# frederik-kofoed-marqversen/quantum_computations

Measured on AMD Instinct MI355X. Metric: gate_apps_per_sec, higher is better.
Workload: dtype f64; 1 GPU; 28-qubit complex128 state vector (28 qubits = 4 GiB per GPU), depth-100 random 1+2-qubit gates (BASELINE.json configs[1], seed 100); n_qubits=28

## Files before the change

quantum_computations_amd/csrc/qsv_api.hip:

```cpp

#include "qsv_internal.h"
#include "qsv_plan.h"

#include <sys/mman.h>

#include <thread>

#include <cmath>
#include <cstring>
#include <vector>

namespace {

thread_local std::string g_last_error;

bool valid(const qsv_state *st) { return st != nullptr; }

inline int bit_of(const qsv_state *st, int q) { return st->n - 1 - q; }

int check_qubits(const qsv_state *st, int k, const int *qs) {
    if (st->kind != 0) return qsv_fail(QSV_ESTATE, "this call needs a qubit register");
    for (int i = 0; i < k; ++i) {
        if (qs[i] < 0) return qsv_fail(QSV_EINVAL, "Non-negative index");
        if (qs[i] >= st->n)
            return qsv_fail(QSV_EINVAL, "qubit index " + std::to_string(qs[i]) + " out of range for a " +
                                            std::to_string(st->n) + "-qubit register");
        for (int j = 0; j < i; ++j)
            if (qs[i] == qs[j]) return qsv_fail(QSV_EINVAL, "Indices must be distinct.");
    }
    return QSV_OK;
}

int alloc_workspace(qsv_state *st) {
    QSV_HIP(hipMalloc(reinterpret_cast<void **>(&st->partials), sizeof(double) * 2 * QSV_REDUCE_BLOCKS));
    QSV_HIP(hipHostMalloc(reinterpret_cast<void **>(&st->partials_host), sizeof(double) * 2 * QSV_REDUCE_BLOCKS,
                          hipHostMallocDefault));
    QSV_HIP(hipEventCreate(&st->ev_start));
    QSV_HIP(hipEventCreate(&st->ev_stop));
    return QSV_OK;
}

int create_common(int kind, int n, int d, uint64_t amps, int device, void *dev_amps, uint64_t capacity,
                  void *stream, qsv_state **out) {
    if (!out) return qsv_fail(QSV_EINVAL, "null output handle");
    *out = nullptr;
    int count = 0;
    hipError_t e = hipGetDeviceCount(&count);
    if (e != hipSuccess || count <= 0)
        return qsv_fail(QSV_EHIP, std::string("no HIP device available: ") +
                                      (e != hipSuccess ? hipGetErrorString(e) : "device count is 0"));
    if (device < 0 || device >= count) return qsv_fail(QSV_EINVAL, "device ordinal out of range");
    QSV_HIP(hipSetDevice(device));
    qsv_state *st = new qsv_state();
    st->device = device;
    st->kind = kind;
    st->n = n;
    st->d = d;
    st->amps = amps;
    st->stream = static_cast<hipStream_t>(stream);
    if (dev_amps) {
        if (capacity < amps) {
            delete st;
            return qsv_fail(QSV_ENOMEM, "view capacity is smaller than the register");
        }
        st->data = static_cast<amp_t *>(dev_amps);
        st->capacity = capacity;
        st->owns_data = false;
    } else {
        if (hipMalloc(reinterpret_cast<void **>(&st->data), sizeof(amp_t) * amps) != hipSuccess) {
            delete st;
            return qsv_fail(QSV_ENOMEM, "device allocation of " + std::to_string(amps * sizeof(amp_t)) +
                                            " bytes for the register failed");
        }
        st->capacity = amps;
        st->owns_data = true;
    }
    int rc = alloc_workspace(st);
    if (rc) {
        qsv_destroy(st);
        return rc;
    }
    if (st->owns_data) {
        rc = qsvk_set_basis(st, 0);
        if (rc) {
            qsv_destroy(st);
            return rc;
        }
    }
    *out = st;
    return QSV_OK;
}

bool is_one(double re, double im) { return re == 1.0 && im == 0.0; }
bool is_zero(double re, double im) { return re == 0.0 && im == 0.0; }

bool matrix_is_diagonal(int D, const double *m) {
    for (int r = 0; r < D; ++r)
        for (int c = 0; c < D; ++c)
            if (r != c && !is_zero(m[2 * (r * D + c)], m[2 * (r * D + c) + 1])) return false;
    return true;
}

bool matrix_equals(int D, const double *m, const double *ref_real) {
    for (int i = 0; i < D * D; ++i)
        if (m[2 * i] != ref_real[i] || m[2 * i + 1] != 0.0) return false;
    return true;
}

constexpr int QSV_MIN_CTRL_BIT = 3;

constexpr int OP_NONE = -1;

QsvOp dense_op(int k, const int *bits, int nctrl, const int *cbits, const double *m) {
    QsvOp op;
    op.kind = QSV_OP_DENSE;
    op.k = k;
    for (int j = 0; j < k; ++j) op.bits[j] = bits[j];
    op.nctrl = nctrl;
    for (int i = 0; i < nctrl; ++i) op.cbits[i] = cbits[i];
    std::memcpy(op.m, m, sizeof(double) * (2u << (2 * k)));
    return op;
}

QsvOp diag_op(int k, const int *bits, int nctrl, const int *cbits, const double *d) {
    QsvOp op;
    op.kind = QSV_OP_DIAG;
    op.k = k;
    for (int j = 0; j < k; ++j) op.bits[j] = bits[j];
    op.nctrl = nctrl;
    for (int i = 0; i < nctrl; ++i) op.cbits[i] = cbits[i];
    std::memcpy(op.m, d, sizeof(double) * (2u << k));
    return op;
}

QsvOp phase_op(int nctrl, const int *cbits, double re, double im) {
    QsvOp op;
    op.kind = QSV_OP_PHASE;
    op.nctrl = nctrl;
    for (int i = 0; i < nctrl; ++i) op.cbits[i] = cbits[i];
    op.m[0] = re;
    op.m[1] = im;
    return op;
}

QsvOp none_op() {
    QsvOp op;
    op.kind = OP_NONE;
    return op;
}

QsvOp diag_1q_bits(qsv_state *st, int bit, const double d[4]) {
    if (st->specialize && is_one(d[0], d[1])) {
        if (is_one(d[2], d[3])) return none_op();
        if (bit >= QSV_MIN_CTRL_BIT) return phase_op(1, &bit, d[2], d[3]);
    }
    return diag_op(1, &bit, 0, nullptr, d);
}

QsvOp diag_2q_bits(qsv_state *st, int b0, int b1, const double d[8]) {
    if (st->specialize) {
        const bool one0 = is_one(d[0], d[1]), one1 = is_one(d[2], d[3]), one2 = is_one(d[4], d[5]);
        const bool c0 = b0 >= QSV_MIN_CTRL_BIT, c1 = b1 >= QSV_MIN_CTRL_BIT;
        if (one0 && one1 && one2) {
            if (is_one(d[6], d[7])) return none_op();
            const double dd[4] = {1.0, 0.0, d[6], d[7]};
            if (c0 && c1) {
                const int both[2] = {b0, b1};
                return phase_op(2, both, d[6], d[7]);
            }
            if (c0) return diag_op(1, &b1, 1, &b0, dd);
            if (c1) return diag_op(1, &b0, 1, &b1, dd);
        } else if (one0 && one1 && c0) {
            return diag_op(1, &b1, 1, &b0, d + 4);
        } else if (one0 && one2 && d[2] == d[6] && d[3] == d[7]) {
            const double dd[4] = {1.0, 0.0, d[2], d[3]};
            return diag_1q_bits(st, b1, dd);
        }
    }
    const int bits[2] = {b0, b1};
    return diag_op(2, bits, 0, nullptr, d);
}

QsvOp controlled_1q_bits(qsv_state *st, int nctrl, const int *cbits, int tbit, const double u[8]) {
    int fold = -1;
    for (int i = 0; i < nctrl && st->n >= QSV_LANE_BITS; ++i)
        if (cbits[i] < QSV_MIN_CTRL_BIT) fold = i;
    if (fold < 0) return dense_op(1, &tbit, nctrl, cbits, u);
    double m[32] = {0};
    m[0] = 1.0;
    m[2 * (1 * 4 + 1)] = 1.0;
    for (int r = 0; r < 2; ++r)
        for (int c = 0; c < 2; ++c) {
            m[2 * ((2 + r) * 4 + 2 + c)] = u[2 * (r * 2 + c)];
            m[2 * ((2 + r) * 4 + 2 + c) + 1] = u[2 * (r * 2 + c) + 1];
        }
    std::vector<int> rest;
    for (int i = 0; i < nctrl; ++i)
        if (i != fold) rest.push_back(cbits[i]);
    const int bits[2] = {cbits[fold], tbit};
    return dense_op(2, bits, static_cast<int>(rest.size()), rest.data(), m);
}

QsvOp swap_bits(qsv_state *st, int b0, int b1) {
    if (b0 >= QSV_LANE_BITS && b1 >= QSV_LANE_BITS && st->n >= QSV_LANE_BITS) {
        QsvOp op;
        op.kind = QSV_OP_PAIR;
        op.k = 2;
// ... 1049 lines not shown
```

quantum_computations_amd/csrc/qsv_internal.h:

```cpp
#pragma once

#include <hip/hip_runtime.h>
#include <stdint.h>

#include <string>
#include <vector>

#include "qsv.h"

typedef double amp_t __attribute__((ext_vector_type(2)));

constexpr int QSV_BLOCK = 256;
constexpr int QSV_LANE_BITS = 6;
constexpr int QSV_MAX_INS = 48;
constexpr int QSV_MAX_K = 6;

struct GateArgs {
    uint64_t W;
    uint64_t or_mask;
    uint64_t hoff[4];
    int32_t nins;
    uint32_t lane_ctrl;
    int32_t remap;
    int32_t ubit;
    int32_t lbit[2];
    int32_t lxor[4];
    uint32_t pos[QSV_MAX_INS];
    double m[32];
};

struct DiagArgs {
    uint64_t W;
    uint64_t or_mask;
    int32_t nins;
    uint32_t lane_ctrl;
    int32_t b0, b1;
    int32_t remap;
    uint32_t pos[QSV_MAX_INS];
    double d[8];
};

enum { QSV_OP_DENSE = 0, QSV_OP_PAIR = 1, QSV_OP_DIAG = 2, QSV_OP_PHASE = 3 };
constexpr int QSV_OP_MAX_CTRL = 40;
struct QsvOp {
    int kind = QSV_OP_DENSE;
    int k = 0;
    int bits[2] = {-1, -1};
    int nctrl = 0;
    int cbits[QSV_OP_MAX_CTRL] = {};
    double m[32] = {};
};

struct qsv_state {
    int device = 0;
    int kind = 0;
    int n = 0;
    int d = 2;
    uint64_t amps = 1;
    uint64_t capacity = 0;
    amp_t *data = nullptr;
    bool owns_data = false;
    amp_t *spare = nullptr;
    uint64_t spare_capacity = 0;
    hipStream_t stream = nullptr;
    double *partials = nullptr;
    double *partials_host = nullptr;
    double *dev_matrix = nullptr;
    size_t dev_matrix_bytes = 0;
    char *stage_host = nullptr;
    char *stage_dev = nullptr;
    hipEvent_t stage_done[8] = {};
    bool stage_busy[8] = {};
    unsigned stage_next = 0;
    hipEvent_t ev_start = nullptr, ev_stop = nullptr;
    std::vector<hipEvent_t> marks;
    int specialize = 1;
    int unroll = 0;
    int grid_cap = 0;
    int nontemporal = 1;
    int ubit = 8;
    int remap = -1;
    int kq_variant = 0;
    int last_passes = 0;
    int tile_sequence_gates = -1;
    int sequence_work = -1;
    int complex_product = 0;
    int readout_variant = 0;
    int plane_kernel = 1;
    char last_kernel[96] = "";
    int defer = -1;
    bool ptr_exposed = false;
    std::vector<QsvOp> queue;
    uint64_t defer_gates = 0;
    uint64_t defer_launches = 0;
};

constexpr int QSV_REDUCE_BLOCKS = 1024;
constexpr int QSV_STAGE_SLOTS = 8;
constexpr size_t QSV_STAGE_BYTES = 512u << 10;

struct StageRef {
    char *dev = nullptr;
    int slot = -1;
};
int qsvk_stage(qsv_state *st, const void *a, size_t bytes_a, const void *b, size_t bytes_b, StageRef *out);
int qsvk_stage_done(qsv_state *st, const StageRef &ref);
inline size_t qsv_pad16(size_t x) { return (x + 15) / 16 * 16; }

int qsv_fail(int code, const std::string &msg);
#define QSV_HIP(expr)                                                                                   \
    do {                                                                                                \
        hipError_t _e = (expr);                                                                         \
        if (_e != hipSuccess)                                                                           \
            return qsv_fail(QSV_EHIP, std::string(#expr) + ": " + hipGetErrorString(_e));               \
    } while (0)

int qsvk_copy(amp_t *dst, const amp_t *src, uint64_t amps, hipStream_t stream);
int qsvk_dense(qsv_state *st, int k, const int *bits, int nctrl, const int *cbits, const double *m_user);
int qsvk_pair_exchange(qsv_state *st, int bit_a, int bit_b);
int qsvk_diag(qsv_state *st, int k, const int *bits, int nctrl, const int *cbits, const double *d_user);
int qsvk_phase(qsv_state *st, int nctrl, const int *cbits, double re, double im);
int qsvk_generic(qsv_state *st, int k, const int *bits, const double *m_user);
int qsvk_sequence5(qsv_state *st, const int *bits, int n_gates, const int *arity, const int *legs, const double *mats);
int qsvk_run_op(qsv_state *st, const QsvOp &op);
int qsvk_pass(qsv_state *st, const QsvOp *const *ops, int count, uint64_t tile_high);
bool qsvk_op_exact(const QsvOp &op);
int qsvk_sequence_tile(qsv_state *st, int k, const int *bits, int n_gates, const int *arity, const int *legs, const double *mats);
constexpr int QSV_UNHANDLED_KQ = 1 << 20;
int qsvk_measure_probs(qsv_state *st, int bit, const double eig0[4], const double eig1[4], double *p0, double *p1);
int qsvk_collapse(qsv_state *st, int bit, const double eig[4], double scale);
int qsvk_insert(qsv_state *st, int bit, const double amp[4]);
int qsvk_permute(qsv_state *st, const int *src_bit_of_dst_bit);
int qsvk_norm2(qsv_state *st, double *out);
int qsvk_inner(qsv_state *a, qsv_state *b, double *re, double *im);
int qsvk_probabilities(qsv_state *st, const uint64_t *indices, int count, double *out);
int qsvk_expect_pauli(qsv_state *st, uint64_t xmask, uint64_t zmask, int n_y, double *re, double *im);
int qsvk_reduced_density(qsv_state *st, int k, const int *bits, double *rho_out);
int qsvk_expect_density(qsv_state *ket, qsv_state *rho, double *re, double *im);
int qsvk_sample(qsv_state *st, int shots, const double *u, uint64_t *out);
int qsvk_fill_random(qsv_state *st, uint64_t seed, uint64_t index_offset, double *norm2);
int qsvk_scale(qsv_state *st, double re, double im);
int qsvk_set_basis(qsv_state *st, uint64_t index);
int qsvk_ensure_matrix(qsv_state *st, size_t bytes);
int qsvk_scratch(qsv_state *st, uint64_t amps, amp_t **out);
int qsvk_adopt(qsv_state *st, uint64_t new_amps);

int qsvq_mode1(qsv_state *st, int mode, const double *m, bool diag);
int qsvq_mode2(qsv_state *st, int mode0, int mode1, const double *m, bool diag);
int qsvq_mode2_gather(qsv_state *st, int mode0, int mode1, int nnz, const int32_t *cols, const double *vals);
int qsvq_mode2_blocks(qsv_state *st, int mode0, int mode1, int nblocks, const int32_t *sizes,
                      const int32_t *plane_indices, const double *mats);
int qsvq_mode_marginal(qsv_state *st, int mode, double *probs);
int qsvq_mode_project(qsv_state *st, int mode, int level, double scale);
int qsvq_mode_insert(qsv_state *st, int mode, const double *vec);
int qsvg_gemm(int device, hipStream_t stream, int op_a, int op_b, uint64_t m, uint64_t n, uint64_t k, const amp_t *a,
              const amp_t *b, amp_t *c);
int qsvg_svd_split(int device, hipStream_t stream, amp_t *theta, uint64_t rows, uint64_t cols, int64_t max_bond_dim,
                   double abs_err, double rel_err, amp_t *m1, amp_t *m2, uint64_t capacity, uint64_t *rank_out,
                   double *s_host);
int qsvg_rsvd_split(int device, hipStream_t stream, const amp_t *theta, uint64_t rows, uint64_t cols, int64_t k_keep,
                    int l, int q, const amp_t *omega, double abs_err, double rel_err, amp_t *m1, amp_t *m2,
                    uint64_t capacity, uint64_t *rank_out, double *s_host);
int qsvg_skinny_gemm(int device, hipStream_t stream, int op, uint64_t n, uint64_t m, int l, const amp_t *A,
                     const amp_t *Q, amp_t *Y);
int qsvg_release_workspace(int device);
int release_retired_probes(int device);
int qsvg_release_stream_workspace(int device, hipStream_t stream);
int qsvg_reserve_workspace(int device, hipStream_t stream, uint64_t bytes);
int qsvq_tensor_scale_axis(int device, hipStream_t stream, amp_t *t, uint64_t L, uint64_t d, uint64_t R,
                           const double *dev_diag);
int qsvq_tensor_plane_diag(int device, hipStream_t stream, amp_t *t, uint64_t L, uint64_t d, uint64_t R,
                           const double *dev_plane);
int qsvq_tensor_plane_gather(int device, hipStream_t stream, const amp_t *in, amp_t *out, uint64_t L, uint64_t d,
                             uint64_t R, int nnz, const int32_t *dev_cols, const double *dev_vals);
int qsvq_tensor_plane_phase(int device, hipStream_t stream, amp_t *t, uint64_t L, uint64_t d, uint64_t R,
                            const double *dev_qs, double strength);
int qsvq_tensor_plane_affine(int device, hipStream_t stream, const amp_t *in, amp_t *out, uint64_t L, uint64_t d,
                             uint64_t R, const double *dev_qs, const double *a);
int qsvq_tensor_outer(int device, hipStream_t stream, const amp_t *p, const amp_t *q, amp_t *out, uint64_t X, uint64_t Y,
                      uint64_t Z, uint64_t W, int swap_last);
int qsvq_tensor_take_level(int device, hipStream_t stream, const amp_t *in, amp_t *out, uint64_t L, uint64_t d,
                           uint64_t R, uint64_t level, double scale);
int qsvq_tensor_insert_axis(int device, hipStream_t stream, const amp_t *in, amp_t *out, uint64_t L, uint64_t d,
                            uint64_t R, const double *dev_vec);
int qsvq_tensor_axis_overlap(int device, hipStream_t stream, const amp_t *z, const amp_t *t, uint64_t L, uint64_t d,
                             uint64_t R, double *dev_out);
int qsvg_axis_gemm(int device, hipStream_t stream, const amp_t *in, amp_t *out, uint64_t L, uint64_t d_in,
                   uint64_t d_out, uint64_t R, const double *dev_m);
int qsvq_tensor_axis_dev(int device, hipStream_t stream, const amp_t *in, amp_t *out, uint64_t L, uint64_t d_in,
                         uint64_t d_out, uint64_t R, const double *dev_m);
int qsvq_tensor_axis(int device, hipStream_t stream, const amp_t *in, amp_t *out, uint64_t L, uint64_t d_in,
                     uint64_t d_out, uint64_t R, const double *m_host);
```

quantum_computations_amd/csrc/qsv_kernels.hip:

```cpp

#include "qsv_internal.h"
#include "qsv_plan.h"

#include <algorithm>
#include <array>
#include <cstdlib>
#include <cstring>
#include <type_traits>
#include <vector>

namespace {

struct cplx {
    double re, im;
};

__device__ __forceinline__ amp_t cmul(cplx m, amp_t a) {
    amp_t r;
    r.x = m.re * a.x - m.im * a.y;
    r.y = m.re * a.y + m.im * a.x;
    return r;
}

__device__ __forceinline__ amp_t cmul_diag(cplx d, amp_t a) {
// ... 2587 lines not shown
    PASS_PAIR = 5,
    PASS_DIAG_T = 6, PASS_DIAG_R1 = 7, PASS_DIAG_R2 = 8, PASS_DIAG_M = 9
};
struct PassGate {
    int32_t form;
    int32_t code;
    uint32_t rc;
    uint32_t tc;
    int32_t tz0, tz1;
    uint64_t omask;
    double m[32];
};
struct PassGroup {
    int32_t first, count;
    int32_t q[4];
    uint64_t gates;
};
constexpr int PASS_TILE = 1 << qsv_plan::TILE_BITS, PASS_ROWS = PASS_TILE / 64, PASS_THREADS = 256;
constexpr int PASS_ROWS_PER_WAVE = PASS_ROWS / (PASS_THREADS / 64);
static_assert(PASS_TILE == PASS_THREADS << qsv_plan::REG_BITS, "one thread per setting of the tile bits outside the registers");

struct PassArgs {
    BigArgs g;
    uint64_t row_off[PASS_ROWS];
};

template <int FORM>
__device__ __forceinline__ constexpr int pass_col(int r, int j) {
    return FORM == 0 ? j : FORM == 1 ? (j ^ r) : (((j & 1) << 1) | ((r & 1) ^ (j >> 1)));
}

struct PassCtl {
    uint32_t rc;
    bool sel;
    bool ok;
};

__device__ __forceinline__ void pass_put(amp_t &x, amp_t y, const PassCtl &ct) {
    if (ct.sel) {
        x.x = ct.ok ? y.x : x.x;
        x.y = ct.ok ? y.y : x.y;
    } else {
        x = y;
    }
}

template <int D, int FORM, int P0, int P1>
__device__ __forceinline__ void pass_dense(amp_t (&x)[16], const double *__restrict__ m, const PassCtl &ct) {
    constexpr int TARGETS = (1 << P0) | (D == 4 ? (1 << P1) : 0);
#pragma unroll
    for (int b = 0; b < 16; ++b) {
        if (b & TARGETS) continue;
        if ((b & ct.rc) != ct.rc) continue;
        int idx[D];
#pragma unroll
        for (int c = 0; c < D; ++c) idx[c] = b | ((c & 1) << P0) | (D == 4 ? ((c >> 1) << P1) : 0);
        amp_t y[D];
#pragma unroll
        for (int r = 0; r < D; ++r) {
            amp_t acc = {0.0, 0.0};
#pragma unroll
            for (int j = 0; j < D; ++j) {
                const int c = pass_col<FORM>(r, j);
                acc = cfma(cplx{m[2 * (r * D + c)], m[2 * (r * D + c) + 1]}, x[idx[c]], acc);
            }
            y[r] = acc;
        }
#pragma unroll
        for (int r = 0; r < D; ++r) pass_put(x[idx[r]], y[r], ct);
    }
}

template <int PA, int PB>
__device__ __forceinline__ void pass_pair(amp_t (&x)[16], const PassCtl &ct) {
#pragma unroll
    for (int b = 0; b < 16; ++b) {
        if (b & ((1 << PA) | (1 << PB))) continue;
        if ((b & ct.rc) != ct.rc) continue;
        const amp_t u = x[b | (1 << PA)], v = x[b | (1 << PB)];
        pass_put(x[b | (1 << PA)], v, ct);
        pass_put(x[b | (1 << PB)], u, ct);
    }
}

template <class Sel>
__device__ __forceinline__ void pass_diag(amp_t (&x)[16], const cplx (&d)[4], const PassCtl &ct, Sel sel) {
#pragma unroll
    for (int c = 0; c < 16; ++c) {
        if ((c & ct.rc) != ct.rc) continue;
        pass_put(x[c], cmul_diag(d[sel(c)], x[c]), ct);
    }
}

__device__ __forceinline__ cplx pass_pick(bool s, cplx one, cplx zero) {
    return cplx{s ? one.re : zero.re, s ? one.im : zero.im};
}

__device__ __forceinline__ void pass_gate16(amp_t (&x)[16], const PassGate &pg, uint32_t g0) {
    const double *__restrict__ m = pg.m;
    const PassCtl ct = {pg.rc, pg.tc != 0, (g0 & pg.tc) == pg.tc};
#define QSV_PASS_D4(FORM, P0, P1) case (FORM) * 16 + (P0) * 4 + (P1): pass_dense<4, (FORM) - PASS_D4, P0, P1>(x, m, ct); break;
#define QSV_PASS_D4_BOTH(FORM, LO, HI) QSV_PASS_D4(FORM, LO, HI) QSV_PASS_D4(FORM, HI, LO)
    switch (pg.form * 16 + pg.code) {
        case PASS_D2 * 16 + 0: pass_dense<2, 0, 0, 0>(x, m, ct); break;
        case PASS_D2 * 16 + 1: pass_dense<2, 0, 1, 0>(x, m, ct); break;
        case PASS_D2 * 16 + 2: pass_dense<2, 0, 2, 0>(x, m, ct); break;
        case PASS_D2 * 16 + 3: pass_dense<2, 0, 3, 0>(x, m, ct); break;
        case PASS_D2X * 16 + 0: pass_dense<2, 1, 0, 0>(x, m, ct); break;
        case PASS_D2X * 16 + 1: pass_dense<2, 1, 1, 0>(x, m, ct); break;
        case PASS_D2X * 16 + 2: pass_dense<2, 1, 2, 0>(x, m, ct); break;
        case PASS_D2X * 16 + 3: pass_dense<2, 1, 3, 0>(x, m, ct); break;
        QSV_PASS_D4_BOTH(PASS_D4, 0, 1) QSV_PASS_D4_BOTH(PASS_D4, 0, 2) QSV_PASS_D4_BOTH(PASS_D4, 0, 3)
        QSV_PASS_D4_BOTH(PASS_D4, 1, 2) QSV_PASS_D4_BOTH(PASS_D4, 1, 3) QSV_PASS_D4_BOTH(PASS_D4, 2, 3)
        QSV_PASS_D4_BOTH(PASS_D4X, 0, 1) QSV_PASS_D4_BOTH(PASS_D4X, 0, 2) QSV_PASS_D4_BOTH(PASS_D4X, 0, 3)
        QSV_PASS_D4_BOTH(PASS_D4X, 1, 2) QSV_PASS_D4_BOTH(PASS_D4X, 1, 3) QSV_PASS_D4_BOTH(PASS_D4X, 2, 3)
        QSV_PASS_D4(PASS_D4HL, 0, 1) QSV_PASS_D4(PASS_D4HL, 0, 2) QSV_PASS_D4(PASS_D4HL, 0, 3)
        QSV_PASS_D4(PASS_D4HL, 1, 2) QSV_PASS_D4(PASS_D4HL, 1, 3) QSV_PASS_D4(PASS_D4HL, 2, 3)
        case PASS_PAIR * 16 + 0 * 4 + 1: pass_pair<0, 1>(x, ct); break;
        case PASS_PAIR * 16 + 0 * 4 + 2: pass_pair<0, 2>(x, ct); break;
        case PASS_PAIR * 16 + 0 * 4 + 3: pass_pair<0, 3>(x, ct); break;
        case PASS_PAIR * 16 + 1 * 4 + 2: pass_pair<1, 2>(x, ct); break;
        case PASS_PAIR * 16 + 1 * 4 + 3: pass_pair<1, 3>(x, ct); break;
        case PASS_PAIR * 16 + 2 * 4 + 3: pass_pair<2, 3>(x, ct); break;
        case PASS_DIAG_T * 16: {
            const bool s0 = (g0 >> pg.tz0) & 1, s1 = (g0 >> pg.tz1) & 1;
            const cplx d[4] = {pass_pick(s0, pass_pick(s1, cplx{m[6], m[7]}, cplx{m[4], m[5]}),
                                         pass_pick(s1, cplx{m[2], m[3]}, cplx{m[0], m[1]})), {}, {}, {}};
            pass_diag(x, d, ct, [](int) { return 0; });
            break;
        }
#define QSV_PASS_R1(P) case PASS_DIAG_R1 * 16 + (P): { \
            const cplx d[4] = {{m[0], m[1]}, {m[2], m[3]}, {}, {}}; \
            pass_diag(x, d, ct, [](int c) { return (c >> (P)) & 1; }); break; }
        QSV_PASS_R1(0) QSV_PASS_R1(1) QSV_PASS_R1(2) QSV_PASS_R1(3)
#define QSV_PASS_R2(P0, P1) case PASS_DIAG_R2 * 16 + (P0) * 4 + (P1): { \
            const cplx d[4] = {{m[0], m[1]}, {m[2], m[3]}, {m[4], m[5]}, {m[6], m[7]}}; \
            pass_diag(x, d, ct, [](int c) { return (((c >> (P0)) & 1) << 1) | ((c >> (P1)) & 1); }); break; }
        QSV_PASS_R2(0, 1) QSV_PASS_R2(0, 2) QSV_PASS_R2(0, 3) QSV_PASS_R2(1, 2) QSV_PASS_R2(1, 3) QSV_PASS_R2(2, 3)
#define QSV_PASS_M(P) case PASS_DIAG_M * 16 + (P): { \
            const bool s = (g0 >> pg.tz0) & 1; \
            const cplx d[4] = {pass_pick(s, cplx{m[2], m[3]}, cplx{m[0], m[1]}), pass_pick(s, cplx{m[6], m[7]}, cplx{m[4], m[5]}), {}, {}}; \
            pass_diag(x, d, ct, [](int c) { return (c >> (P)) & 1; }); break; }
        QSV_PASS_M(0) QSV_PASS_M(1) QSV_PASS_M(2) QSV_PASS_M(3)
        default: break;
    }
#undef QSV_PASS_D4
#undef QSV_PASS_D4_BOTH
#undef QSV_PASS_R1
#undef QSV_PASS_R2
#undef QSV_PASS_M
}

template <bool NT>
__global__ __launch_bounds__(PASS_THREADS) void k_pass_tile(amp_t *__restrict__ a, const PassArgs pa,
                                                            const PassGate *__restrict__ gates, int n_gates,
                                                            const PassGroup *__restrict__ groups, int n_groups) {
    __shared__ amp_t tile[PASS_TILE];
    const BigArgs &g = pa.g;
    const int lane = threadIdx.x & 63;
    const int q = __builtin_amdgcn_readfirstlane(threadIdx.x >> 6);
    constexpr int RPW = PASS_ROWS_PER_WAVE;
    const uint64_t tile_id = (g.regions > 1 && gridDim.x % g.regions == 0)
                                 ? (blockIdx.x % g.regions) * (gridDim.x / g.regions) + blockIdx.x / g.regions
                                 : blockIdx.x;
    const uint64_t base = deposit(g.w0 + tile_id, g);
    uint64_t active = 0;
    for (int i = 0; i < n_gates; ++i)
        if ((base & gates[i].omask) == gates[i].omask) active |= 1ull << i;
    if (!active) return;
#if defined(__HIP_DEVICE_COMPILE__)
#pragma unroll
    for (int i = 0; i < RPW; ++i)
        __builtin_amdgcn_global_load_lds(a + base + pa.row_off[q * RPW + i] + lane, tile + (q * RPW + i) * 64, 16, 0, NT ? 2 : 0);
#endif
    __syncthreads();
#pragma unroll 1
    for (int p = 0; p < n_groups; ++p) {
        const PassGroup &gr = groups[p];
        if (!(active & gr.gates)) continue;
        const int q0 = gr.q[0], q1 = gr.q[1], q2 = gr.q[2], q3 = gr.q[3];
        uint32_t g0 = threadIdx.x;
        g0 = static_cast<uint32_t>(insert_zero(g0, q0));
        g0 = static_cast<uint32_t>(insert_zero(g0, q1));
        g0 = static_cast<uint32_t>(insert_zero(g0, q2));
        g0 = static_cast<uint32_t>(insert_zero(g0, q3));
        amp_t x[16];
#pragma unroll
        for (int c = 0; c < 16; ++c)
            x[c] = tile[g0 | ((c & 1) << q0) | (((c >> 1) & 1) << q1) | (((c >> 2) & 1) << q2) | (((c >> 3) & 1) << q3)];
#pragma unroll 1
        for (int i = gr.first; i < gr.first + gr.count; ++i)
            if ((active >> i) & 1) pass_gate16(x, gates[i], g0);
#pragma unroll
        for (int c = 0; c < 16; ++c)
            tile[g0 | ((c & 1) << q0) | (((c >> 1) & 1) << q1) | (((c >> 2) & 1) << q2) | (((c >> 3) & 1) << q3)] = x[c];
        __syncthreads();
    }
#pragma unroll
    for (int i = 0; i < RPW; ++i) st<NT>(a + base + pa.row_off[q * RPW + i] + lane, tile[(q * RPW + i) * 64 + lane]);
}

bool qsvk_op_exact(const QsvOp &op) {
    if (op.kind == QSV_OP_PAIR) return true;
    auto unit = [](double re, double im) { return im == 0.0 && (re == 1.0 || re == -1.0); };
    if (op.kind == QSV_OP_PHASE) return unit(op.m[0], op.m[1]);
    if (op.kind == QSV_OP_DIAG) {
        for (int i = 0; i < (1 << op.k); ++i)
            if (!unit(op.m[2 * i], op.m[2 * i + 1])) return false;
        return true;
    }
    const int D = 1 << op.k;
    int per_col[4] = {0, 0, 0, 0};
    for (int r = 0; r < D; ++r) {
        int nz = 0;
        for (int c = 0; c < D; ++c) {
            const double re = op.m[2 * (r * D + c)], im = op.m[2 * (r * D + c) + 1];
            if (re == 0.0 && im == 0.0) continue;
            if (!unit(re, im)) return false;
            ++nz;
            ++per_col[c];
        }
        if (nz != 1) return false;
    }
    for (int c = 0; c < D; ++c)
        if (per_col[c] != 1) return false;
    return true;
}

int qsvk_run_op(qsv_state *st, const QsvOp &op) {
    switch (op.kind) {
        case QSV_OP_DENSE: return qsvk_dense(st, op.k, op.bits, op.nctrl, op.cbits, op.m);
        case QSV_OP_PAIR: return qsvk_pair_exchange(st, op.bits[0], op.bits[1]);
        case QSV_OP_DIAG: return qsvk_diag(st, op.k, op.bits, op.nctrl, op.cbits, op.m);
        case QSV_OP_PHASE: return qsvk_phase(st, op.nctrl, op.cbits, op.m[0], op.m[1]);
        default: return qsv_fail(QSV_EINVAL, "internal: unknown queued gate kind");
    }
}

int qsvk_pass(qsv_state *st, const QsvOp *const *ops, int count, uint64_t tile_high) {
    const uint64_t low = (1ull << QSV_LANE_BITS) - 1;
    if (count < 1 || count > qsv_plan::MAX_PASS_GATES || st->n < qsv_plan::TILE_BITS || (tile_high & low) ||
        __builtin_popcountll(tile_high) != qsv_plan::HIGH_BITS || (tile_high >> st->n))
        return qsv_fail(QSV_EINVAL, "internal: malformed gate pass");
    int tile_bits[qsv_plan::TILE_BITS];
    int local_of[64];
    for (int b = 0; b < 64; ++b) {
        local_of[b] = qsv_plan::tile_index(b, tile_high);
        if (local_of[b] >= 0) tile_bits[local_of[b]] = b;
    }
    std::vector<PassGate> rec(count);
    std::vector<std::array<int, 2>> leg(count, std::array<int, 2>{-1, -1});
    std::vector<uint32_t> cmask(count, 0), need(count, 0);
    for (int i = 0; i < count; ++i) {
        const QsvOp &op = *ops[i];
        PassGate &pg = rec[i];
        std::memset(&pg, 0, sizeof(pg));
        uint64_t ctrl = 0;
        for (int c = 0; c < op.nctrl; ++c) ctrl |= 1ull << op.cbits[c];
        const qsv_plan::ControlMasks cm = qsv_plan::control_masks(ctrl, tile_high);
        cmask[i] = cm.inside;
        pg.omask = cm.outside;
        for (int j = 0; j < op.k; ++j)
            if (local_of[op.bits[j]] < 0) return qsv_fail(QSV_EINVAL, "internal: gate target outside its pass's tile");
        if (op.kind == QSV_OP_DIAG || op.kind == QSV_OP_PHASE) {
            pg.form = PASS_DIAG_T;
            if (op.kind == QSV_OP_PHASE) {
                for (int e = 0; e < 4; ++e) {
                    pg.m[2 * e] = op.m[0];
                    pg.m[2 * e + 1] = op.m[1];
                }
            } else {
                leg[i][0] = local_of[op.bits[0]];
                if (op.k == 2) leg[i][1] = local_of[op.bits[1]];
                std::memcpy(pg.m, op.m, sizeof(double) * (2u << op.k));
            }
            continue;
        }
        if (op.kind == QSV_OP_PAIR) {
            pg.form = PASS_PAIR;
            leg[i] = {local_of[op.bits[0]], local_of[op.bits[1]]};
            need[i] = (1u << leg[i][0]) | (1u << leg[i][1]);
            continue;
        }
        const int k = op.k, D = 1 << k;
        int kb[2] = {op.bits[0], op.bits[1]};
        int form;
        if (tile12_takes(st, k, op.bits, op.nctrl, op.cbits)) {
            form = k == 1 ? PASS_D2 : PASS_D4;
        } else {
            int low_b[2], high_b[2], nl = 0, nh = 0;
            for (int j = 0; j < k; ++j) {
                if (op.bits[j] >= QSV_LANE_BITS) high_b[nh++] = op.bits[j];
                else low_b[nl++] = op.bits[j];
            }
            for (int j = 0; j < nl; ++j) kb[j] = low_b[j];
            for (int j = 0; j < nh; ++j) kb[nl + j] = high_b[j];
            form = nl == 0 ? (k == 1 ? PASS_D2 : PASS_D4) : nh == 0 ? (k == 1 ? PASS_D2X : PASS_D4X) : PASS_D4HL;
        }
        pg.form = form;
        auto user_index = [&](int kidx) {
            int u = 0;
            for (int i2 = 0; i2 < k; ++i2) {
                const int bitval = (kidx >> i2) & 1;
                for (int j = 0; j < k; ++j)
                    if (op.bits[j] == kb[i2]) u |= bitval << (k - 1 - j);
            }
            return u;
        };
        for (int r = 0; r < D; ++r)
            for (int c = 0; c < D; ++c) {
                const int ur = user_index(r), uc = user_index(c);
                pg.m[2 * (r * D + c)] = op.m[2 * (ur * D + uc)];
                pg.m[2 * (r * D + c) + 1] = op.m[2 * (ur * D + uc) + 1];
            }
        for (int i2 = 0; i2 < k; ++i2) {
            leg[i][i2] = local_of[kb[i2]];
            need[i] |= 1u << leg[i][i2];
        }
    }
    const std::vector<qsv_plan::Group> cut = qsv_plan::cut_groups(need);
    std::vector<PassGroup> grp(cut.size());
    for (size_t p = 0; p < cut.size(); ++p) {
        PassGroup &gr = grp[p];
        std::memset(&gr, 0, sizeof(gr));
        gr.first = cut[p].first;
        gr.count = cut[p].count;
        int reg_of[qsv_plan::TILE_BITS];
        for (int t = 0; t < qsv_plan::TILE_BITS; ++t) reg_of[t] = -1;
        for (int j = 0; j < qsv_plan::REG_BITS; ++j) {
            gr.q[j] = cut[p].reg[j];
            reg_of[gr.q[j]] = j;
        }
        for (int i = gr.first; i < gr.first + gr.count; ++i) {
            PassGate &pg = rec[i];
            gr.gates |= 1ull << i;
            for (int t = 0; t < qsv_plan::TILE_BITS; ++t)
                if ((cmask[i] >> t) & 1) {
                    if (reg_of[t] >= 0) pg.rc |= 1u << reg_of[t];
                    else pg.tc |= 1u << t;
                }
            const int l0 = leg[i][0], l1 = leg[i][1];
            if (pg.form == PASS_DIAG_T) {
                const int r0 = l0 >= 0 ? reg_of[l0] : -1, r1 = l1 >= 0 ? reg_of[l1] : -1;
                auto swap_d1_d2 = [&pg]() {
                    std::swap(pg.m[2], pg.m[4]);
                    std::swap(pg.m[3], pg.m[5]);
                };
                if (l0 < 0) {
                    pg.tz0 = pg.tz1 = 0;
                } else if (l1 < 0) {
                    if (r0 >= 0) {
                        pg.form = PASS_DIAG_R1;
                        pg.code = r0;
                    } else {
                        pg.m[6] = pg.m[2];
                        pg.m[7] = pg.m[3];
                        pg.tz0 = pg.tz1 = l0;
                    }
                } else if (r0 >= 0 && r1 >= 0) {
                    pg.form = PASS_DIAG_R2;
                    if (r0 > r1) swap_d1_d2();
                    pg.code = std::min(r0, r1) * 4 + std::max(r0, r1);
                } else if (r0 >= 0 || r1 >= 0) {
                    pg.form = PASS_DIAG_M;
                    if (r0 < 0) swap_d1_d2();
                    pg.code = r0 >= 0 ? r0 : r1;
                    pg.tz0 = r0 >= 0 ? l1 : l0;
                } else {
                    pg.tz0 = l0;
                    pg.tz1 = l1;
                }
                continue;
            }
            const int r0 = reg_of[l0], r1 = l1 >= 0 ? reg_of[l1] : 0;
            if (r0 < 0 || r1 < 0) return qsv_fail(QSV_EINVAL, "internal: gate target outside its group's register bits");
            if (pg.form == PASS_PAIR) pg.code = std::min(r0, r1) * 4 + std::max(r0, r1);
            else if (pg.form == PASS_D2 || pg.form == PASS_D2X) pg.code = r0;
            else pg.code = r0 * 4 + r1;
        }
    }
    StageRef staged;
    int rc = qsvk_stage(st, rec.data(), sizeof(PassGate) * rec.size(), grp.data(), sizeof(PassGroup) * grp.size(), &staged);
    if (rc) return rc;
    const PassGate *dev_g = reinterpret_cast<const PassGate *>(staged.dev);
    const PassGroup *dev_p = reinterpret_cast<const PassGroup *>(staged.dev + qsv_pad16(sizeof(PassGate) * rec.size()));
    const int n_groups = static_cast<int>(grp.size());
    PassArgs pa;
    std::memset(&pa, 0, sizeof(pa));
    BigArgs &g = pa.g;
    g.W = st->amps >> qsv_plan::TILE_BITS;
    g.nins = qsv_plan::TILE_BITS;
    for (int j = 0; j < qsv_plan::TILE_BITS; ++j) g.pos[j] = static_cast<uint32_t>(tile_bits[j]);
    for (int row = 0; row < PASS_ROWS; ++row)
        for (int j = 0; j < qsv_plan::HIGH_BITS; ++j)
            if ((row >> j) & 1) pa.row_off[row] |= 1ull << tile_bits[QSV_LANE_BITS + j];
    g.regions = st->remap >= 0 ? static_cast<uint32_t>(st->remap) : 8;
    const bool nt = st->nontemporal != 0;
    snprintf(st->last_kernel, sizeof(st->last_kernel), "k_pass_tile<%s>", nt ? "true" : "false");
    const uint64_t per_launch = 1ull << 23;
    for (g.w0 = 0; g.w0 < g.W; g.w0 += per_launch) {
        const dim3 gd(static_cast<unsigned>(std::min(per_launch, g.W - g.w0))), bd(PASS_THREADS);
        if (nt) hipLaunchKernelGGL(k_pass_tile<true>, gd, bd, 0, st->stream, st->data, pa, dev_g, count, dev_p, n_groups);
        else hipLaunchKernelGGL(k_pass_tile<false>, gd, bd, 0, st->stream, st->data, pa, dev_g, count, dev_p, n_groups);
        rc = check_launch();
        if (rc) return rc;
    }
    return qsvk_stage_done(st, staged);
}

static int launch_dense_mfma(qsv_state *st, int k, const int *bits, const double *m_user) {
    const int D = 1 << k;
    const std::vector<int> tb(bits, bits + k);
    std::vector<int> sorted(tb);
    std::sort(sorted.begin(), sorted.end());
    std::vector<uint64_t> off(D, 0);
    for (int c = 0; c < D; ++c)
        for (int i = 0; i < k; ++i)
            if ((c >> i) & 1) off[c] |= 1ull << sorted[i];
    auto user_index = [&](int c) {
        int u = 0;
        for (int leg = 0; leg < k; ++leg)
            for (int i = 0; i < k; ++i)
                if (sorted[i] == tb[leg]) u |= ((c >> i) & 1) << (k - 1 - leg);
        return u;
    };
    bool real_matrix = true;
    for (int i = 0; i < D * D && real_matrix; ++i) real_matrix = m_user[2 * i + 1] == 0.0;
    std::vector<double> m(real_matrix ? D * D : 2 * D * D);
    std::vector<int> ui(D);
    for (int c = 0; c < D; ++c) ui[c] = user_index(c);
    for (int r = 0; r < D; ++r)
        for (int c = 0; c < D; ++c) {
            const int ur = ui[r], uc = ui[c];
            m[c * D + r] = m_user[2 * (ur * D + uc)];
            if (!real_matrix) m[D * D + c * D + r] = m_user[2 * (ur * D + uc) + 1];
        }
    StageRef staged;
    int rc = qsvk_stage(st, m.data(), sizeof(double) * m.size(), off.data(), sizeof(uint64_t) * D, &staged);
    if (rc) return rc;
    const double *dev_m = reinterpret_cast<const double *>(staged.dev);
    const uint64_t *dev_off = reinterpret_cast<const uint64_t *>(staged.dev + qsv_pad16(sizeof(double) * m.size()));
    Mfma6Args g;
    std::memset(&g, 0, sizeof(g));
    g.W = st->amps >> k;
    g.nins = k;
    for (int i = 0; i < k; ++i) g.pos[i] = static_cast<uint32_t>(sorted[i]);
    const bool nt = st->nontemporal != 0;
    const size_t lds = sizeof(double) * (real_matrix ? 1 : 2) * D * D + sizeof(uint64_t) * D;
    int cus = 256;
    (void)hipDeviceGetAttribute(&cus, hipDeviceAttributeMultiprocessorCount, st->device);
    const uint64_t wave_tiles = g.W / 16;
    const unsigned grid = static_cast<unsigned>(std::min<uint64_t>((wave_tiles + 3) / 4, ((k == 6 && !real_matrix) ? 2ull : 3ull) * cus));
    const bool m3 = !real_matrix && st->complex_product != 4;
    snprintf(st->last_kernel, sizeof(st->last_kernel), "k_dense_mfma<%d, %s, %s%s>", k, nt ? "true" : "false",
             real_matrix ? "true" : "false", m3 ? ", true" : "");
#define QSV_LAUNCH_MFMA(KK, N, ...)                                                                                \
    do {                                                                                                           \
        QSV_HIP(hipFuncSetAttribute(reinterpret_cast<const void *>(k_dense_mfma<KK, N, __VA_ARGS__>),              \
                                    hipFuncAttributeMaxDynamicSharedMemorySize, static_cast<int>(lds)));           \
        hipLaunchKernelGGL((k_dense_mfma<KK, N, __VA_ARGS__>), dim3(grid), dim3(QSV_BLOCK), lds, st->stream,       \
                           st->data, g, dev_m, dev_off);                                                           \
    } while (0)
    if (k == 6 && m3) {
        if (nt) QSV_LAUNCH_MFMA(6, true, false, true);
        else QSV_LAUNCH_MFMA(6, false, false, true);
    } else if (k == 6) {
        if (nt) { if (real_matrix) QSV_LAUNCH_MFMA(6, true, true); else QSV_LAUNCH_MFMA(6, true, false); }
        else { if (real_matrix) QSV_LAUNCH_MFMA(6, false, true); else QSV_LAUNCH_MFMA(6, false, false); }
    } else if (m3) {
        if (nt) QSV_LAUNCH_MFMA(5, true, false, true);
        else QSV_LAUNCH_MFMA(5, false, false, true);
    } else {
        if (nt) { if (real_matrix) QSV_LAUNCH_MFMA(5, true, true); else QSV_LAUNCH_MFMA(5, true, false); }
        else { if (real_matrix) QSV_LAUNCH_MFMA(5, false, true); else QSV_LAUNCH_MFMA(5, false, false); }
    }
#undef QSV_LAUNCH_MFMA
    rc = check_launch();
    if (rc) return rc;
    return qsvk_stage_done(st, staged);
}

int qsvk_generic(qsv_state *st, int k, const int *bits, const double *m_user) {
    if (k < 1 || k > QSV_MAX_K) return qsv_fail(QSV_EINVAL, "generic gate: k must be in 1..6");
    const bool mfma_ok = st->n >= k && (st->amps >> k) >= 16;
    if (k == 6 && mfma_ok && st->kq_variant == 0) return launch_dense_mfma(st, 6, bits, m_user);
    if (k == 5 && mfma_ok && st->kq_variant == 5) return launch_dense_mfma(st, 5, bits, m_user);
    if (k >= 3 && k <= 6 && st->n >= k) {
        const int rc_big = launch_dense_big(st, k, bits, m_user);
        if (rc_big != QSV_UNHANDLED_KQ) return rc_big;
    }
    const size_t bytes = sizeof(double) * 2ull << (2 * k);
    StageRef staged;
    int rc = qsvk_stage(st, m_user, bytes, nullptr, 0, &staged);
    if (rc) return rc;
    const double *dev_m = reinterpret_cast<const double *>(staged.dev);
    GenericArgs g;
    std::memset(&g, 0, sizeof(g));
    g.K = k;
    g.W = st->amps >> k;
    std::vector<int> sorted(bits, bits + k);
    std::sort(sorted.begin(), sorted.end());
    for (int j = 0; j < k; ++j) {
        g.sorted_pos[j] = static_cast<uint8_t>(sorted[j]);
        g.leg_pos[j] = static_cast<uint8_t>(bits[j]);
    }
    const int grid = grid_for(g.W, QSV_BLOCK, 4096);
    snprintf(st->last_kernel, sizeof(st->last_kernel), "k_generic<%d>", k);
    switch (k) {
        case 1: hipLaunchKernelGGL((k_generic<1>), dim3(grid), dim3(QSV_BLOCK), 0, st->stream, st->data, g, dev_m); break;
        case 2: hipLaunchKernelGGL((k_generic<2>), dim3(grid), dim3(QSV_BLOCK), 0, st->stream, st->data, g, dev_m); break;
        case 3: hipLaunchKernelGGL((k_generic<3>), dim3(grid), dim3(QSV_BLOCK), 0, st->stream, st->data, g, dev_m); break;
        case 4: hipLaunchKernelGGL((k_generic<4>), dim3(grid), dim3(QSV_BLOCK), 0, st->stream, st->data, g, dev_m); break;
        case 5: hipLaunchKernelGGL((k_generic<5>), dim3(grid), dim3(QSV_BLOCK), 0, st->stream, st->data, g, dev_m); break;
        default: hipLaunchKernelGGL((k_generic<6>), dim3(grid), dim3(QSV_BLOCK), 0, st->stream, st->data, g, dev_m); break;
    }
    rc = check_launch();
    if (rc) return rc;
    return qsvk_stage_done(st, staged);
}

int qsvk_dense(qsv_state *st, int k, const int *bits, int nctrl, const int *cbits, const double *m_user) {
    if (k < 1 || k > 2) return qsv_fail(QSV_EINVAL, "dense kernel handles 1- and 2-qubit matrices");
    if (st->n < QSV_LANE_BITS) {
        if (nctrl == 0) return qsvk_generic(st, k, bits, m_user);
        std::vector<int> legs(cbits, cbits + nctrl);
        legs.insert(legs.end(), bits, bits + k);
        const std::vector<double> full = expand_controls(k, nctrl, m_user);
        return qsvk_generic(st, k + nctrl, legs.data(), full.data());
    }
    if (st->unroll == 0 && st->kq_variant != 1 && st->kq_variant != 2) {
        const int rc_tile = launch_tile12(st, k, bits, nctrl, cbits, m_user);
        if (rc_tile != QSV_UNHANDLED_KQ) return rc_tile;
    }
    GateArgs g;
    std::memset(&g, 0, sizeof(g));
    std::vector<int> high, low;
    for (int j = 0; j < k; ++j) (bits[j] >= QSV_LANE_BITS ? high : low).push_back(bits[j]);
    const int KH = static_cast<int>(high.size()), KL = static_cast<int>(low.size());
    int rc = fill_enumeration(st, g, high, nctrl, cbits);
    if (rc) return rc;
    for (int h = 0; h < (1 << KH); ++h) {
        uint64_t o = 0;
        for (int i = 0; i < KH; ++i)
            if ((h >> i) & 1) o |= 1ull << high[i];
        g.hoff[h] = o;
    }
    for (int j = 0; j < KL; ++j) g.lbit[j] = low[j];
    for (int x = 0; x < (1 << KL); ++x) {
        int mask = 0;
        for (int j = 0; j < KL; ++j)
            if ((x >> j) & 1) mask |= 1 << low[j];
        g.lxor[x] = mask;
    }
    const int D = 1 << k;
    auto user_index = [&](int kidx) {
        const int h = kidx >> KL, l = kidx & ((1 << KL) - 1);
        int u = 0;
        for (int j = 0; j < k; ++j) {
            int bitval = 0;
// ... 530 lines not shown
```

quantum_computations_amd/csrc/qsv_plan.h:

```cpp
#pragma once

#include <stdint.h>

#include <vector>

namespace qsv_plan {

constexpr int TILE_BITS = 12;
constexpr int LANE_BITS = 6;
constexpr int HIGH_BITS = TILE_BITS - LANE_BITS;
constexpr int MAX_PASS_GATES = 64;
constexpr uint64_t LOW_MASK = (1ull << LANE_BITS) - 1;

constexpr int REG_BITS = 4;

constexpr float PASS_BASE = 1.0f;
constexpr float PASS_PER_GROUP = 0.12f;
constexpr float PASS_PER_GATE = 0.08f;

struct Gate {
    uint64_t need = 0;
    uint64_t ctrl = 0;
    bool exact = false;
    float cost = 1.0f;
    bool dense = true;
};

struct Pass {
    uint64_t tile = 0;
    std::vector<int> gates;
    bool fused = false;
};

inline int popcount64(uint64_t x) { return __builtin_popcountll(x); }

inline int tile_index(int b, uint64_t tile) {
    if (b < LANE_BITS) return b;
    if (b >= 64 || !((tile >> b) & 1)) return -1;
    return LANE_BITS + popcount64(tile & ((1ull << b) - 1));
}

struct ControlMasks {
    uint32_t inside = 0;
    uint64_t outside = 0;
};
inline ControlMasks control_masks(uint64_t ctrl, uint64_t tile) {
    ControlMasks cm;
    for (int b = 0; b < 64; ++b) {
        if (!((ctrl >> b) & 1)) continue;
        const int t = tile_index(b, tile);
        if (t >= 0) cm.inside |= 1u << t;
        else cm.outside |= 1ull << b;
    }
    return cm;
}

inline float active_fraction(const std::vector<Gate> &q, const std::vector<int> &gates, uint64_t tile) {
    float frac = 0.0f;
    for (int i : gates) {
        const int outside = popcount64(q[i].ctrl & ~tile & ~LOW_MASK);
        frac += 1.0f / static_cast<float>(1ull << (outside < 60 ? outside : 60));
        if (frac >= 1.0f) return 1.0f;
    }
    return frac;
}

struct Group {
    int first = 0, count = 0;
    int reg[REG_BITS] = {0, 0, 0, 0};
};

inline std::vector<Group> cut_groups(const std::vector<uint32_t> &need, int tile_bits = TILE_BITS) {
    std::vector<Group> out;
    std::vector<uint32_t> masks;
    uint32_t cur = 0;
    for (int i = 0; i < static_cast<int>(need.size()); ++i) {
        const uint32_t grown = cur | need[i];
        if (out.empty() || popcount64(grown) > REG_BITS) {
            if (!out.empty()) masks.push_back(cur);
            Group g;
            g.first = i;
            out.push_back(g);
            cur = need[i];
        } else {
            cur = grown;
        }
        ++out.back().count;
    }
    if (!out.empty()) masks.push_back(cur);
    for (size_t k = 0; k < out.size(); ++k) {
        uint32_t m = masks[k];
        for (int t = tile_bits - 1; t >= 0 && popcount64(m) < REG_BITS; --t)
            if (!((m >> t) & 1)) m |= 1u << t;
        int w = 0;
        for (int t = 0; t < tile_bits && w < REG_BITS; ++t)
            if ((m >> t) & 1) out[k].reg[w++] = t;
    }
    return out;
}

inline uint32_t need_in_tile(uint64_t need, uint64_t tile) {
    uint32_t m = 0;
    for (int b = 0; b < 64; ++b)
        if ((need >> b) & 1) {
            const int t = tile_index(b, tile);
            if (t >= 0) m |= 1u << t;
        }
    return m;
}

inline int count_groups(const std::vector<Gate> &q, const std::vector<int> &gates, uint64_t tile) {
    std::vector<uint32_t> need;
    need.reserve(gates.size());
    for (int i : gates) need.push_back(q[i].dense ? need_in_tile(q[i].need, tile) : 0u);
    return static_cast<int>(cut_groups(need).size());
}

inline float pass_cost(const std::vector<Gate> &q, const std::vector<int> &gates, uint64_t tile) {
    return PASS_BASE * active_fraction(q, gates, tile) + PASS_PER_GROUP * static_cast<float>(count_groups(q, gates, tile)) +
           PASS_PER_GATE * static_cast<float>(gates.size());
}

inline Pass plan_first(const std::vector<Gate> &q, int n) {
    Pass p;
    if (q.empty()) return p;
    const uint64_t all = n >= 64 ? ~0ull : (1ull << n) - 1;
    const int high_bits = n - LANE_BITS < HIGH_BITS ? n - LANE_BITS : HIGH_BITS;
    uint64_t tile = 0, blocked = 0;
    bool left_behind = false;
    for (int i = 0; i < static_cast<int>(q.size()) && static_cast<int>(p.gates.size()) < MAX_PASS_GATES; ++i) {
        const Gate &g = q[i];
        const uint64_t bits = g.need | g.ctrl;
        const bool order_ok = !left_behind || (g.exact && (bits & blocked) == 0);
        const uint64_t grown = tile | (g.need & ~LOW_MASK);
        if (order_ok && popcount64(grown) <= high_bits) {
            tile = grown;
            p.gates.push_back(i);
        } else {
            left_behind = true;
            blocked |= bits;
        }
    }
    for (int b = LANE_BITS; b < n && popcount64(tile) < high_bits; ++b)
        if (!((tile >> b) & 1)) tile |= 1ull << b;
    p.tile = tile & all;
    float alone = 0.0f;
    for (int i : p.gates) alone += q[i].cost;
    p.fused = p.gates.size() >= 2 && pass_cost(q, p.gates, p.tile) < alone;
    if (!p.fused) p.gates.resize(1);
    return p;
}

inline std::vector<Pass> plan_stream(const std::vector<Gate> &q, int n, size_t window) {
    std::vector<Pass> out;
    std::vector<Gate> pending;
    std::vector<int> idx;
    auto launch_first = [&]() {
        Pass p = plan_first(pending, n);
        std::vector<bool> taken(pending.size(), false);
        for (int &i : p.gates) {
            taken[i] = true;
            i = idx[i];
        }
        size_t w = 0;
        for (size_t i = 0; i < pending.size(); ++i)
            if (!taken[i]) {
                pending[w] = pending[i];
                idx[w++] = idx[i];
            }
        pending.resize(w);
        idx.resize(w);
        out.push_back(std::move(p));
    };
    for (size_t i = 0; i < q.size(); ++i) {
        pending.push_back(q[i]);
        idx.push_back(static_cast<int>(i));
        if (pending.size() >= window) launch_first();
    }
    while (!pending.empty()) launch_first();
    return out;
}

}
```

Before: 4331 gate-apps/s.

## Make fused pass kernel persistent with software-prefetched next tile

Replaces the one-block-per-tile launch of the fused pass kernel with a persistent grid sized at two blocks per CU, and each block walks its tiles in a strided loop. While a block applies gates to the current tile in LDS, the next active tile is prefetched into registers, overlapping global loads with compute. The per-tile active-gate mask is now computed with a wave ballot. Inactive tiles are skipped during the walk. Risks include extra register pressure from the prefetch buffer, a sync added after every group, and the loss of the parallelism that came from launching many blocks.

```diff
diff --git a/quantum_computations_amd/csrc/qsv_api.hip b/quantum_computations_amd/csrc/qsv_api.hip
--- a/quantum_computations_amd/csrc/qsv_api.hip
+++ b/quantum_computations_amd/csrc/qsv_api.hip
@@ -53,6 +53,8 @@
     QSV_HIP(hipSetDevice(device));
     qsv_state *st = new qsv_state();
     st->device = device;
+    if (hipDeviceGetAttribute(&st->cus, hipDeviceAttributeMultiprocessorCount, device) != hipSuccess || st->cus < 1)
+        st->cus = 256;
     st->kind = kind;
     st->n = n;
     st->d = d;
diff --git a/quantum_computations_amd/csrc/qsv_internal.h b/quantum_computations_amd/csrc/qsv_internal.h
--- a/quantum_computations_amd/csrc/qsv_internal.h
+++ b/quantum_computations_amd/csrc/qsv_internal.h
@@ -53,6 +53,7 @@
 
 struct qsv_state {
     int device = 0;
+    int cus = 256;
     int kind = 0;
     int n = 0;
     int d = 2;
diff --git a/quantum_computations_amd/csrc/qsv_kernels.hip b/quantum_computations_amd/csrc/qsv_kernels.hip
--- a/quantum_computations_amd/csrc/qsv_kernels.hip
+++ b/quantum_computations_amd/csrc/qsv_kernels.hip
@@ -2763,52 +2763,69 @@
 }
 
 template <bool NT>
-__global__ __launch_bounds__(PASS_THREADS) void k_pass_tile(amp_t *__restrict__ a, const PassArgs pa,
-                                                            const PassGate *__restrict__ gates, int n_gates,
-                                                            const PassGroup *__restrict__ groups, int n_groups) {
+__global__ __launch_bounds__(PASS_THREADS, 2) void k_pass_tile(amp_t *__restrict__ a, const PassArgs pa,
+                                                               const PassGate *__restrict__ gates, int n_gates,
+                                                               const PassGroup *__restrict__ groups, int n_groups) {
     __shared__ amp_t tile[PASS_TILE];
     const BigArgs &g = pa.g;
     const int lane = threadIdx.x & 63;
     const int q = __builtin_amdgcn_readfirstlane(threadIdx.x >> 6);
     constexpr int RPW = PASS_ROWS_PER_WAVE;
-    const uint64_t tile_id = (g.regions > 1 && gridDim.x % g.regions == 0)
-                                 ? (blockIdx.x % g.regions) * (gridDim.x / g.regions) + blockIdx.x / g.regions
-                                 : blockIdx.x;
-    const uint64_t base = deposit(g.w0 + tile_id, g);
-    uint64_t active = 0;
-    for (int i = 0; i < n_gates; ++i)
-        if ((base & gates[i].omask) == gates[i].omask) active |= 1ull << i;
-    if (!active) return;
+    const uint64_t omask = lane < n_gates ? gates[lane].omask : ~0ull;
+    uint64_t next_base = 0, next_active = 0;
+    auto acts = [&](uint64_t t) {
+        next_base = deposit(t, g);
+        next_active = __ballot((next_base & omask) == omask);
+        return next_active != 0;
+    };
+    const uint64_t tiles = g.W, grid = gridDim.x;
+    uint64_t s = qsv_plan::walk_next(blockIdx.x, grid, tiles, g.regions, acts);
+    if (s >= tiles) return;
 #if defined(__HIP_DEVICE_COMPILE__)
 #pragma unroll
     for (int i = 0; i < RPW; ++i)
-        __builtin_amdgcn_global_load_lds(a + base + pa.row_off[q * RPW + i] + lane, tile + (q * RPW + i) * 64, 16, 0, NT ? 2 : 0);
+        __builtin_amdgcn_global_load_lds(a + next_base + pa.row_off[q * RPW + i] + lane, tile + (q * RPW + i) * 64, 16, 0, NT ? 2 : 0);
 #endif
     __syncthreads();
+    for (;;) {
+        const uint64_t base = next_base;
+        const uint64_t active = next_active;
+        s = qsv_plan::walk_next(s + grid, grid, tiles, g.regions, acts);
+        const bool more = s < tiles;
+        amp_t pre[RPW];
+        if (more) {
+#pragma unroll
+            for (int i = 0; i < RPW; ++i) pre[i] = ld<NT>(a + next_base + pa.row_off[q * RPW + i] + lane);
+        }
 #pragma unroll 1
-    for (int p = 0; p < n_groups; ++p) {
-        const PassGroup &gr = groups[p];
-        if (!(active & gr.gates)) continue;
-        const int q0 = gr.q[0], q1 = gr.q[1], q2 = gr.q[2], q3 = gr.q[3];
-        uint32_t g0 = threadIdx.x;
-        g0 = static_cast<uint32_t>(insert_zero(g0, q0));
-        g0 = static_cast<uint32_t>(insert_zero(g0, q1));
-        g0 = static_cast<uint32_t>(insert_zero(g0, q2));
-        g0 = static_cast<uint32_t>(insert_zero(g0, q3));
-        amp_t x[16];
-#pragma unroll
-        for (int c = 0; c < 16; ++c)
-            x[c] = tile[g0 | ((c & 1) << q0) | (((c >> 1) & 1) << q1) | (((c >> 2) & 1) << q2) | (((c >> 3) & 1) << q3)];
+        for (int p = 0; p < n_groups; ++p) {
+            const PassGroup &gr = groups[p];
+            if (!(active & gr.gates)) continue;
+            const int q0 = gr.q[0], q1 = gr.q[1], q2 = gr.q[2], q3 = gr.q[3];
+            uint32_t g0 = threadIdx.x;
+            g0 = static_cast<uint32_t>(insert_zero(g0, q0));
+            g0 = static_cast<uint32_t>(insert_zero(g0, q1));
+            g0 = static_cast<uint32_t>(insert_zero(g0, q2));
+            g0 = static_cast<uint32_t>(insert_zero(g0, q3));
+            amp_t x[16];
+#pragma unroll
+            for (int c = 0; c < 16; ++c)
+                x[c] = tile[g0 | ((c & 1) << q0) | (((c >> 1) & 1) << q1) | (((c >> 2) & 1) << q2) | (((c >> 3) & 1) << q3)];
 #pragma unroll 1
-        for (int i = gr.first; i < gr.first + gr.count; ++i)
-            if ((active >> i) & 1) pass_gate16(x, gates[i], g0);
-#pragma unroll
-        for (int c = 0; c < 16; ++c)
-            tile[g0 | ((c & 1) << q0) | (((c >> 1) & 1) << q1) | (((c >> 2) & 1) << q2) | (((c >> 3) & 1) << q3)] = x[c];
+            for (int i = gr.first; i < gr.first + gr.count; ++i)
+                if ((active >> i) & 1) pass_gate16(x, gates[i], g0);
+#pragma unroll
+            for (int c = 0; c < 16; ++c)
+                tile[g0 | ((c & 1) << q0) | (((c >> 1) & 1) << q1) | (((c >> 2) & 1) << q2) | (((c >> 3) & 1) << q3)] = x[c];
+            __syncthreads();
+        }
+#pragma unroll
+        for (int i = 0; i < RPW; ++i) st<NT>(a + base + pa.row_off[q * RPW + i] + lane, tile[(q * RPW + i) * 64 + lane]);
+        if (!more) break;
+#pragma unroll
+        for (int i = 0; i < RPW; ++i) tile[(q * RPW + i) * 64 + lane] = pre[i];
         __syncthreads();
     }
-#pragma unroll
-    for (int i = 0; i < RPW; ++i) st<NT>(a + base + pa.row_off[q * RPW + i] + lane, tile[(q * RPW + i) * 64 + lane]);
 }
 
 bool qsvk_op_exact(const QsvOp &op) {
@@ -3008,14 +3025,13 @@
     g.regions = st->remap >= 0 ? static_cast<uint32_t>(st->remap) : 8;
     const bool nt = st->nontemporal != 0;
     snprintf(st->last_kernel, sizeof(st->last_kernel), "k_pass_tile<%s>", nt ? "true" : "false");
-    const uint64_t per_launch = 1ull << 23;
-    for (g.w0 = 0; g.w0 < g.W; g.w0 += per_launch) {
-        const dim3 gd(static_cast<unsigned>(std::min(per_launch, g.W - g.w0))), bd(PASS_THREADS);
-        if (nt) hipLaunchKernelGGL(k_pass_tile<true>, gd, bd, 0, st->stream, st->data, pa, dev_g, count, dev_p, n_groups);
-        else hipLaunchKernelGGL(k_pass_tile<false>, gd, bd, 0, st->stream, st->data, pa, dev_g, count, dev_p, n_groups);
-        rc = check_launch();
-        if (rc) return rc;
-    }
+    uint64_t grid = std::min<uint64_t>(g.W, 2ull * static_cast<uint64_t>(st->cus));
+    if (st->grid_cap > 0) grid = std::min<uint64_t>(grid, static_cast<uint64_t>(st->grid_cap));
+    const dim3 gd(static_cast<unsigned>(grid)), bd(PASS_THREADS);
+    if (nt) hipLaunchKernelGGL(k_pass_tile<true>, gd, bd, 0, st->stream, st->data, pa, dev_g, count, dev_p, n_groups);
+    else hipLaunchKernelGGL(k_pass_tile<false>, gd, bd, 0, st->stream, st->data, pa, dev_g, count, dev_p, n_groups);
+    rc = check_launch();
+    if (rc) return rc;
     return qsvk_stage_done(st, staged);
 }
 
diff --git a/quantum_computations_amd/csrc/qsv_plan.h b/quantum_computations_amd/csrc/qsv_plan.h
--- a/quantum_computations_amd/csrc/qsv_plan.h
+++ b/quantum_computations_amd/csrc/qsv_plan.h
@@ -119,6 +119,23 @@
 inline float pass_cost(const std::vector<Gate> &q, const std::vector<int> &gates, uint64_t tile) {
     return PASS_BASE * active_fraction(q, gates, tile) + PASS_PER_GROUP * static_cast<float>(count_groups(q, gates, tile)) +
            PASS_PER_GATE * static_cast<float>(gates.size());
+}
+
+#if defined(__HIPCC__)
+#define QSV_PLAN_HD __host__ __device__
+#else
+#define QSV_PLAN_HD
+#endif
+
+QSV_PLAN_HD inline uint64_t walk_tile(uint64_t s, uint64_t tiles, uint32_t regions) {
+    return (regions > 1 && tiles % regions == 0) ? (s % regions) * (tiles / regions) + s / regions : s;
+}
+
+template <class Active>
+QSV_PLAN_HD inline uint64_t walk_next(uint64_t s, uint64_t grid, uint64_t tiles, uint32_t regions, Active &&active) {
+    for (; s < tiles; s += grid)
+        if (active(walk_tile(s, tiles, regions))) return s;
+    return tiles;
 }
 
 inline Pass plan_first(const std::vector<Gate> &q, int n) {
```

Result: slower. 4040 gate-apps/s (-6.7%).
